# ardaduz/deep-video-mvs

Hardware: AMD Instinct MI355X
Metric: depth frames/sec/GPU @ 320x256x64 planes (fusionnet); rel-L1 vs ref (higher is better)
Workload: dtype f32

## Files before the change

### deep-video-mvs_amd/csrc/direct_conv.hip

```cpp
#include <stdlib.h>

#include "dvmvs_device.h"

namespace dvmvs {

typedef float float4v __attribute__((ext_vector_type(4)));

struct DirectConvArgs {
  const float* x;
  const float* packed;
  const float* bias;
  float* dst;
  float* dst_nhwc;
  long long x_batch_stride, dst_batch_stride;
  int B, C_in, C_out, H, W, OH, OW;
  int act;
  int n_groups;
  int packed_groups;
  int n_chunks;
  int tiles_x;
  int vec4;
};

#ifdef DVMVS_SWEEP_TRACE
constexpr int kDcTraceWords = 8, kDcTraceWaves = 16384;
// ... 308 lines not shown
  packed[i] = (kx < K && co < C_out && ci < C_in) ? w[((static_cast<size_t>(co) * C_in + ci) * K + ky) * K + kx] : 0.0f;
}

__device__ inline float head_activation(float v, int act, float p0, float p1) {
#pragma clang fp contract(off)
  if (act == 1) return fmaxf(v, 0.0f);
  if (act == 2 || act == 3) {
    const float s = 1.0f / (1.0f + expf(-v));
    return act == 2 ? s : 1.0f / (p0 * s + p1);
  }
  return v;
}

template <int PX>
__global__ __launch_bounds__(256) void conv_head_kernel(const float* __restrict__ x, const float* __restrict__ w, const float* __restrict__ bias,
                                                        float* __restrict__ dst, long long x_batch_stride, long long dst_batch_stride, int C, int H,
                                                        int W, int act, float p0, float p1) {
  constexpr int SL = 256 / PX;
  __shared__ float s_part[SL][PX];
  const int px = threadIdx.x % PX, slice = threadIdx.x / PX;
  const int HW = H * W;
  const int p = blockIdx.x * PX + px, b = blockIdx.y;
  const int y = p / W, xx = p - y * W;
  const int per = (C + SL - 1) / SL;
  const int c_lo = slice * per, c_hi = min(C, c_lo + per);
  float sum = 0.0f;
  if (p < HW) {
    int off[9];
    bool in[9];
#pragma unroll
    for (int t = 0; t < 9; ++t) {
      const int yy = y + t / 3 - 1, xs = xx + t % 3 - 1;
      in[t] = yy >= 0 && yy < H && xs >= 0 && xs < W;
      off[t] = in[t] ? yy * W + xs : 0;
    }
    const float* xb = x + static_cast<size_t>(b) * x_batch_stride;
#pragma unroll 2
    for (int c = c_lo; c < c_hi; ++c) {
      const float* plane = xb + static_cast<size_t>(c) * HW;
      float v[9];
#pragma unroll
      for (int t = 0; t < 9; ++t) v[t] = in[t] ? plane[off[t]] : 0.0f;
#pragma unroll
      for (int t = 0; t < 9; ++t) sum = fmaf(v[t], w[c * 9 + t], sum);
    }
  }
  s_part[slice][px] = sum;
  __syncthreads();
  if (slice == 0 && p < HW) {
    float total = s_part[0][px];
#pragma unroll
    for (int s = 1; s < SL; ++s) total += s_part[s][px];
    if (bias) total += bias[0];
    dst[static_cast<size_t>(b) * dst_batch_stride + p] = head_activation(total, act, p0, p1);
  }
}

struct DirectConvShape {
  int MW, MT, NT, PW, KS;
};
constexpr DirectConvShape kDcShapes[4] = {{16, 5, 2, 4, 2}, {8, 5, 2, 1, 8}, {16, 5, 1, 1, 8}, {8, 5, 1, 1, 8}};
constexpr int kDcCUs = 256;

inline int direct_conv_choose(int B, int C_in, int C_out, int H, int W, int K, int S) {
  if (B <= 0 || C_in <= 0 || C_out <= 0 || C_out % 16 != 0 || (K != 3 && K != 5) || (S != 1 && S != 2) || H <= 0 || W <= 0) return 0;
  if (S == 2 && (H % 2 != 0 || W % 2 != 0)) return 0;
  const int OH = H / S, OW = W / S;
#if defined(DVMVS_SWEEP_TUNING)
  const char* f = getenv("DVMVS_DC_SHAPE");
  const int forced = f ? atoi(f) : 0;
#else
  const int forced = 0;
#endif
  int best = 0;
  double best_fill = 0.0;
// ... 94 lines not shown
  a.dst_batch_stride = dst_batch_stride ? dst_batch_stride : static_cast<long long>(C_out) * a.OH * a.OW;
  if (a.x_batch_stride < static_cast<long long>(C_in) * H * W || a.dst_batch_stride < static_cast<long long>(C_out) * a.OH * a.OW) return DVMVS_EINVAL;
  if (W % 4 != 0 || a.x_batch_stride % 4 != 0 || (reinterpret_cast<uintptr_t>(x) & 15) != 0) return DVMVS_EUNSUPPORTED;
  if (static_cast<long long>(C_in + 64) * H * W * 4 >= (1LL << 31)) return DVMVS_EUNSUPPORTED;
  a.act = activation;
  a.n_groups = (C_in + 3) / 4;
  a.packed_groups = dc_packed_groups(C_in);
  a.vec4 = (a.OW % 4 == 0 && (a.OH * a.OW) % 4 == 0 && a.dst_batch_stride % 4 == 0 && (reinterpret_cast<uintptr_t>(dst) & 15) == 0) ? 1 : 0;
  a.n_chunks = 0; a.tiles_x = 0;
  hipStream_t s = static_cast<hipStream_t>(stream);
  if (kernel_size == 3) return stride == 1 ? launch_direct_conv_shape<3, 1>(id, a, s) : launch_direct_conv_shape<3, 2>(id, a, s);
  return stride == 1 ? launch_direct_conv_shape<5, 1>(id, a, s) : launch_direct_conv_shape<5, 2>(id, a, s);
}

extern "C" int dvmvs_conv_head_fwd(const float* x, long long x_batch_stride, const float* weight, const float* bias, float* dst,
                                   long long dst_batch_stride, int B, int C_in, int H, int W, int activation, float p0, float p1, dvmvs_stream_t stream) {
  using namespace dvmvs;
  if (!x || !weight || !dst || B <= 0 || C_in <= 0 || H <= 0 || W <= 0) return DVMVS_EINVAL;
  if (activation < 0 || activation > 3) return DVMVS_EINVAL;
  const long long HW = static_cast<long long>(H) * W;
  if (x_batch_stride == 0) x_batch_stride = HW * C_in;
  if (dst_batch_stride == 0) dst_batch_stride = HW;
  hipStream_t s = static_cast<hipStream_t>(stream);
  if (HW >= 16384) {
    hipLaunchKernelGGL((conv_head_kernel<64>), dim3(static_cast<unsigned int>((HW + 63) / 64), B), dim3(256), 0, s, x, weight, bias, dst, x_batch_stride,
                       dst_batch_stride, C_in, H, W, activation, p0, p1);
  } else {
    hipLaunchKernelGGL((conv_head_kernel<16>), dim3(static_cast<unsigned int>((HW + 15) / 16), B), dim3(256), 0, s, x, weight, bias, dst, x_batch_stride,
                       dst_batch_stride, C_in, H, W, activation, p0, p1);
  }
  return launch_status();
}

#ifdef DVMVS_SWEEP_TRACE
extern "C" int dvmvs_debug_direct_conv_trace(unsigned long long* host, int waves) {
  if (waves > dvmvs::kDcTraceWaves) waves = dvmvs::kDcTraceWaves;
  return static_cast<int>(hipMemcpyFromSymbol(host, HIP_SYMBOL(dvmvs::g_dc_trace), sizeof(unsigned long long) * dvmvs::kDcTraceWords * waves));
}
#endif
```

### deep-video-mvs_amd/csrc/frame_ops.hip

```cpp
#include "dvmvs_device.h"

namespace dvmvs {

template <int ACT>
__device__ inline float apply_act(float v, float p0 = 0.0f, float p1 = 0.0f) {
  if (ACT == 1) return fmaxf(v, 0.0f);
  if (ACT == 2) return 1.0f / (1.0f + expf(-v));
  if (ACT == 3) {
#pragma clang fp contract(off)
    const float s = 1.0f / (1.0f + expf(-v));
    return 1.0f / (p0 * s + p1);
  }
  return v;
}

template <int ACT, bool VEC4, int RES>
__global__ __launch_bounds__(256) void bias_act_kernel(const float* x, float* dst, long long dst_batch_stride, const float* __restrict__ bias,
                                                       const float* __restrict__ residual, int C, int HW, int W, float p0, float p1) {
  const int plane = blockIdx.y;
  const int b = plane / C, c = plane - b * C;
  const float bv = bias ? bias[c] : 0.0f;
  const float* p = x + static_cast<size_t>(plane) * HW;
  float* d = dst + static_cast<size_t>(b) * dst_batch_stride + static_cast<size_t>(c) * HW;
  if (VEC4 && RES != 2) {
// ... 86 lines not shown
      const float v00 = PRE ? apply_act<PRE>(r0[x0] + bv) : r0[x0], v01 = PRE ? apply_act<PRE>(r0[x1] + bv) : r0[x1];
      const float v10 = PRE ? apply_act<PRE>(r1[x0] + bv) : r1[x0], v11 = PRE ? apply_act<PRE>(r1[x1] + bv) : r1[x1];
      v[e] = h0 * (w0 * v00 + w1 * v01) + h1 * (w0 * v10 + w1 * v11);
    }
    *reinterpret_cast<float4v*>(dst + oy * OW + ox) = v;
  }
}

template <int PRE>
__global__ __launch_bounds__(256) void upsample2x_quads_kernel(const float* __restrict__ in, float* __restrict__ out, long long out_batch_stride,
                                                               const float* __restrict__ pre_bias, int C, int H, int W) {
  upsample2x_quads_plane<PRE>(in, out, out_batch_stride, pre_bias, blockIdx.y, C, H, W);
}

template <int PRE2>
__global__ __launch_bounds__(256) void upsample2x_pair_quads_kernel(const float* __restrict__ in1, float* __restrict__ out1, long long out1_batch_stride, int C1,
                                                                    const float* __restrict__ in2, float* __restrict__ out2, long long out2_batch_stride,
                                                                    const float* __restrict__ pre_bias2, int C2, int planes1, int H, int W) {
  const int pl = blockIdx.y;
  if (pl < planes1) upsample2x_quads_plane<0>(in1, out1, out1_batch_stride, nullptr, pl, C1, H, W);
  else upsample2x_quads_plane<PRE2>(in2, out2, out2_batch_stride, pre_bias2, pl - planes1, C2, H, W);
}

template <int K, int ACT, bool PRE>
__global__ __launch_bounds__(256) void depthwise_conv_kernel(const float* __restrict__ in, const float* __restrict__ weight,
                                                             const float* __restrict__ bias, const float* __restrict__ pre_bias,
                                                             float* __restrict__ out, int C, int H, int W, int OH, int OW, int stride) {
  const int c = blockIdx.y, b = blockIdx.z;
  const float* wk = weight + static_cast<size_t>(c) * K * K;
  const float* src = in + (static_cast<size_t>(b) * C + c) * H * W;
  float* dst = out + (static_cast<size_t>(b) * C + c) * OH * OW;
  const float bv = bias ? bias[c] : 0.0f;
  const float pv = (PRE && pre_bias) ? pre_bias[c] : 0.0f;
  for (int i = blockIdx.x * blockDim.x + threadIdx.x; i < OH * OW; i += gridDim.x * blockDim.x) {
    const int oy = i / OW, ox = i - oy * OW;
    const int y0 = oy * stride - K / 2, x0 = ox * stride - K / 2;
    float acc = 0.0f;
#pragma unroll
    for (int ky = 0; ky < K; ++ky) {
      const int y = y0 + ky;
      const bool yin = y >= 0 && y < H;
#pragma unroll
      for (int kx = 0; kx < K; ++kx) {
        const int x = x0 + kx;
        float v = 0.0f;
        if (yin && x >= 0 && x < W) v = PRE ? fmaxf(src[y * W + x] + pv, 0.0f) : src[y * W + x];
// ... 126 lines not shown
  using namespace dvmvs;
  if (!in1 || !out1 || !in2 || !out2 || B <= 0 || C1 <= 0 || C2 <= 0 || H <= 0 || W <= 0) return DVMVS_EINVAL;
  if (pre_activation2 < 0 || pre_activation2 > 2) return DVMVS_EINVAL;
  if (out1_batch_stride == 0) out1_batch_stride = static_cast<long long>(C1) * H * W * 4;
  if (out2_batch_stride == 0) out2_batch_stride = static_cast<long long>(C2) * H * W * 4;
  if (out1_batch_stride < static_cast<long long>(C1) * H * W * 4 || out2_batch_stride < static_cast<long long>(C2) * H * W * 4) return DVMVS_EINVAL;
  const long long planes = static_cast<long long>(B) * (C1 + C2);
  const bool quads = W % 2 == 0 && ((reinterpret_cast<uintptr_t>(out1) | reinterpret_cast<uintptr_t>(out2)) & 15) == 0 && ((out1_batch_stride | out2_batch_stride) & 3) == 0 &&
                     planes <= 65535 && static_cast<long long>(H) * W < (1LL << 27);
  if (!quads) {
    const int rc = dvmvs_upsample2x_fwd(in1, out1, out1_batch_stride, nullptr, 0, B, C1, H, W, stream);
    return rc != 0 ? rc : dvmvs_upsample2x_fwd(in2, out2, out2_batch_stride, pre_bias2, pre_activation2, B, C2, H, W, stream);
  }
  const int n_quads = 2 * H * (W / 2);
  const int per_plane = max(1, min((n_quads + 255) / 256, max(1, 4096 / static_cast<int>(planes))));
  const dim3 grid(static_cast<unsigned>(per_plane), static_cast<unsigned>(planes)), block(256);
  hipStream_t s = static_cast<hipStream_t>(stream);
#define DVMVS_UP2(P) hipLaunchKernelGGL(upsample2x_pair_quads_kernel<P>, grid, block, 0, s, in1, out1, out1_batch_stride, C1, in2, out2, out2_batch_stride, pre_bias2, C2, B * C1, H, W)
  if (pre_activation2 == 1) DVMVS_UP2(1); else if (pre_activation2 == 2) DVMVS_UP2(2); else DVMVS_UP2(0);
#undef DVMVS_UP2
  return launch_status();
}

extern "C" int dvmvs_depthwise_conv_fwd(const float* in, const float* weight, const float* bias, const float* pre_bias, int pre_relu,
                                        float* out, int B, int C, int H, int W, int kernel_size, int stride, int activation,
                                        dvmvs_stream_t stream) {
  using namespace dvmvs;
  if (!in || !weight || !out || B <= 0 || C <= 0 || H <= 0 || W <= 0) return DVMVS_EINVAL;
  if ((kernel_size != 3 && kernel_size != 5) || (stride != 1 && stride != 2) || activation < 0 || activation > 2) return DVMVS_EUNSUPPORTED;
  if (C > 65535 || B > 65535) return DVMVS_EUNSUPPORTED;
  const int pad = kernel_size / 2;
  const int OH = (H + 2 * pad - kernel_size) / stride + 1, OW = (W + 2 * pad - kernel_size) / stride + 1;
  hipStream_t s = static_cast<hipStream_t>(stream);
#define DVMVS_DW(K, A) return launch_depthwise<K, A>(in, weight, bias, pre_bias, pre_relu != 0, out, B, C, H, W, OH, OW, stride, s)
  if (kernel_size == 3) {
    if (activation == 0) DVMVS_DW(3, 0);
    if (activation == 1) DVMVS_DW(3, 1);
    DVMVS_DW(3, 2);
  }
  if (activation == 0) DVMVS_DW(5, 0);
  if (activation == 1) DVMVS_DW(5, 1);
  DVMVS_DW(5, 2);
#undef DVMVS_DW
}

extern "C" int dvmvs_nchw_to_nhwc(const float* src, float* dst, int B, int C, int H, int W, dvmvs_stream_t stream) {
// ... 27 lines not shown
```

### deep-video-mvs_amd/dvmvs/engine.py

```python
import contextlib
import copy
import time
import os
from collections import OrderedDict
from typing import NamedTuple

import torch
from torch import nn

from dvmvs.config import Config
from dvmvs.hip import ops as _ops
from dvmvs import pose_algebra as _pose_algebra
from dvmvs import utils as _utils

import dvmvs as _package
_DETERMINISTIC_MIOPEN = _package.DETERMINISTIC_MIOPEN
_MIOPEN_SWITCH_WAS_PRESET = _package.MIOPEN_SWITCH_WAS_PRESET or os.environ.get("DVMVS_KEEP_MIOPEN_ATOMIC_KERNELS", "0") == "1"

_MAX_MEAS = 8
_STAGING_SLOTS = int(os.environ.get("DVMVS_STAGING_SLOTS", "1"))
_GRAPH_QUEUE_FILLERS = int(os.environ.get("DVMVS_GRAPH_QUEUE_FILLERS", "1"))
def _fork_point(value):
    try:
        level = int(value)
# ... 575 lines not shown
        self.step_clock = None
        self._parity, self._prefetched = 0, None
        self._side_stream = torch.cuda.Stream(device=self.device)
        self._aux_stream = torch.cuda.Stream(device=self.device) if _AUX_STREAM != "0" else None
        self._planner, self._planned, self._param_host_ahead = None, None, None
        self.plan_frames_ahead = os.environ.get("DVMVS_PLAN_AHEAD", "1") != "0"
        self.planned_frames_used = 0
        self.ring_wait_seconds = 0.0
        self.lookahead_rejected = 0
        self._switch_interval_before = None
        self._filler_buffers, self._filler_graphs = None, []
        self._copies = CopyQueue()
        self._staging_seen = {}
        self.warm_captured_graphs = os.environ.get("DVMVS_WARM_GRAPHS", "1") != "0"
        self.warm_graph_launches = max(1, int(os.environ.get("DVMVS_WARM_GRAPH_LAUNCHES", "3")))
        if max_lookahead is None:
            max_lookahead = int(os.environ.get("DVMVS_LOOKAHEAD", "1"))
        self.max_lookahead = max(0, min(2, int(max_lookahead)))
        self.warmup_seconds = {"eager_first_frames": 0.0, "graph_capture": 0.0, "graph_first_launches": 0.0}
        self.warmup_graphs_launched = 0
        self.lstm_gates_on_partials = os.environ.get("DVMVS_LSTM_GATES_ON_PARTIALS", "1") != "0"
        self.sweep_variant_counts = {}
        self.sweep_work_list = bool(_utils.SWEEP_WORK_LIST and self.pose_algebra == "reference" and _utils.COST_VOLUME_VARIANT in (0, 2, 3, 4, 5))
        self.sweep_mfma = bool(self.direct and self.sweep_work_list and _utils.COST_VOLUME_VARIANT == 0 and os.environ.get("DVMVS_SWEEP_MFMA", "1") != "0"
                               and (self.height // 2) * (self.width // 2) >= 64 * 64)
        self._tiled_variants = (6,) if self.sweep_mfma else (2, 3, 4, 5)
        self._feature_cache = FeatureCache(self.cache_size, self.device, self.sweep_mfma)
        self.reset()

    def conv_plan_report(self):
        rows = []
        for m in (self.fe, self.fs, self.enc, self.lstm, self.dec):
            for sub in ([] if m is None else m.modules()):
                if isinstance(sub, FusedConv2d):
                    rows += [(shape, tuple(sub.weight.shape)) + tuple(plan) for shape, plan in sub.plans.items()]
        return rows

    @property
    def is_fusionnet(self):
        return self.lstm is not None

    def reset(self, sequence=None):
        if sequence is None or self.sequences == 1:
            self.has_previous = False
            self._no_previous[:] = True
            if self._static is not None:
# ... 256 lines not shown
        self._param_host.copy_(self._param_host_ahead)
        self.planned_frames_used += 1
        return result

    def _fpn_direct(self, taps, outs, half_nhwc=None):
        fpn = self.fs.fpn
        top = fpn.inner_blocks[-1](taps[-1])
        for level in range(len(taps) - 2, -1, -1):
            top = fpn.inner_blocks[level](taps[level], residual=top, residual_mode=2)
            if level == 0 and half_nhwc is not None and isinstance(fpn.layer_blocks[0], FusedConv2d):
                fpn.layer_blocks[0](top, out=outs[0], out_nhwc=half_nhwc)
                half_nhwc = None
            else:
                fpn.layer_blocks[level](top, out=outs[level])
        if half_nhwc is not None:
            _ops.nchw_to_nhwc_into(outs[0], half_nhwc)

    def _decoder_block_direct(self, block, x, cat, depth_head, depth_input):
        up_channels = block.up_convolution.conv[0].weight.shape[0]
        up_conv = block.up_convolution.conv[0]
        if depth_head is not None and _PAIRED_UPSAMPLING and self._aux_stream is None:
            B, C, H, W = x.shape
            up = torch.empty((B, C, 2 * H, 2 * W), device=x.device, dtype=torch.float32)
            _ops.upsample2x_pair_into(x, up, depth_head[0](depth_input, raw=True), cat[:, -1:], depth_head[0].bias, _ops.ACTIVATIONS["sigmoid"])
            up_conv(up, out=cat[:, :up_channels])
            return block.convolution2[0](block.convolution1[0](cat))
        if depth_head is not None:
            with self._beside("heads"):
                self._upsampled_depth_head(depth_head, depth_input, cat[:, -1:])
        if isinstance(up_conv, FusedConv2d):
            up_conv.forward_upsampled(x, out=cat[:, :up_channels])
        else:
            up_conv(_ops.upsample2x(x), out=cat[:, :up_channels])
        self._join_beside()
        return block.convolution2[0](block.convolution1[0](cat))

    @contextlib.contextmanager
    def _beside(self, use):
        aux = self._aux_stream if _AUX_STREAM in ("1", use) else None
        if aux is None:
            yield
            return
        aux.wait_stream(torch.cuda.current_stream(self.device))
        with torch.cuda.stream(aux):
            yield
        self._beside_open = True

    def _join_beside(self):
        if self._aux_stream is not None and getattr(self, "_beside_open", False):
            torch.cuda.current_stream(self.device).wait_stream(self._aux_stream)
            self._beside_open = False

    @staticmethod
    def _upsampled_depth_head(head, x, dst):
        _ops.upsample2x_into(head[0](x, raw=True), dst, head[0].bias, _ops.ACTIVATIONS["sigmoid"])

    def _lstm_bottleneck(self, x):
        if not self.bottleneck_convs:
# ... 121 lines not shown
            cell = self.lstm.lstm_cell
            if not state_warped:
                self._state_warp_direct(buffers, has_previous)
            self._join_beside()
            if self._lstm_bottleneck(lstm_cat):
                splits = _ops.bottleneck_conv_into(lstm_cat, self._lstm_packed, cell.conv.weight.shape[0], 1, self._lstm_partials)
                if self.lstm_gates_on_partials:
                    _ops.lstm_gates_partials_into(self._lstm_partials, splits, s["c"], s["h"])
                else:
                    _ops.partial_sums_bias_act_into(self._lstm_partials, splits, self._lstm_combined, None, _ops.ACTIVATIONS["none"],
                                                    tuple(self._lstm_combined.shape))
                    _ops.lstm_gates_into(self._lstm_combined, s["c"], s["h"])
            else:
                combined = cell.conv(lstm_cat)
                if not combined.is_contiguous():
                    combined = combined.contiguous()
                _ops.lstm_gates_into(combined, s["c"], s["h"])
            bottom = s["h"]
        d1 = self._decoder_block_direct(dec.decoder_block1, bottom, dec_cat[0], None, None)
        d2 = self._decoder_block_direct(dec.decoder_block2, d1, dec_cat[1], dec.depth_layer_one_sixteen, d1)
        d3 = self._decoder_block_direct(dec.decoder_block3, d2, dec_cat[2], dec.depth_layer_one_eight, d2)
        d4 = self._decoder_block_direct(dec.decoder_block4, d3, dec_cat[3], dec.depth_layer_quarter, d3)
        full_in = buffers["full_in"]
        if _PAIRED_UPSAMPLING and self._aux_stream is None:
            _ops.upsample2x_pair_into(d4, full_in[:, :32], dec.depth_layer_half[0](d4, raw=True), full_in[:, 32:33], dec.depth_layer_half[0].bias,
                                      _ops.ACTIVATIONS["sigmoid"])
        else:
            with self._beside("heads"):
                self._upsampled_depth_head(dec.depth_layer_half, d4, full_in[:, 32:33])
            _ops.upsample2x_into(d4, full_in[:, :32])
            self._join_beside()
        refined = dec.refine[1][0](dec.refine[0][0](full_in))
        dec.depth_layer_full[0](refined, out=s["prev_depth"], activation=_ops.ACTIVATION_SIGMOID_TO_DEPTH,
                                p0=dec.inverse_depth_multiplier, p1=dec.inverse_depth_base)

    def _frame_body(self, n_meas, has_previous, sweep_variant=0, parity=0, have=0, give=0, n_meas_next=0, next_variant=0):
        if self.direct:
            return self._frame_body_direct(n_meas, has_previous, sweep_variant, parity, have, give, n_meas_next, next_variant)
        s = self._static
        feats = self._features(s["image"])
        ref_half = feats[0].contiguous()
        s["ref_half"].copy_(ref_half)
        Hm, kt = self._sweep_views(n_meas)
        exact = self.pose_algebra == "exact"
        if exact:
            Hm, kt = _ops.sweep_matrices(s["pose"], s["meas_pose"][:n_meas], s["half_K"])
        cost_volume = _ops.cost_volume(ref_half, s["meas_feat"][:n_meas], Hm, kt, self.min_depth, self.max_depth, self.n_depth_levels,
# ... 269 lines not shown
```

### deep-video-mvs_amd/dvmvs/hip/_capi.py

```python
import ctypes
import os
import threading

import torch

_HERE = os.path.dirname(os.path.abspath(__file__))
LIB_PATH = os.environ.get("DVMVS_HIP_LIB", os.path.normpath(os.path.join(_HERE, "..", "..", "lib", "libdvmvs_hip.so")))

ABI_VERSION = 11
MAX_MEASUREMENTS = 8
MAX_DEPTH_LEVELS = 256
LAYOUT_NCHW, LAYOUT_NHWC = 0, 1

_c_fp = ctypes.c_void_p
_c_fpp = ctypes.POINTER(ctypes.c_void_p)
_c_int = ctypes.c_int
_c_dbl = ctypes.c_double
_c_stream = ctypes.c_void_p
_c_f3 = ctypes.POINTER(ctypes.c_float)

SIGNATURES = {
    "dvmvs_abi_version": (_c_int, []),
    "dvmvs_build_arch": (ctypes.c_char_p, []),
    "dvmvs_error_string": (ctypes.c_char_p, [_c_int]),
# ... 69 lines not shown
    "dvmvs_gp_filter_step": (_c_int, [_c_fp, _c_fp, _c_fp, _c_int, _c_dbl, _c_dbl, _c_dbl, _c_dbl, _c_dbl, _c_dbl, _c_int, _c_stream]),
    "dvmvs_dps_volume_fwd": (_c_int, [_c_fp, _c_fp, _c_fp, _c_fp, _c_fp, _c_fp, _c_int, _c_int, _c_int, _c_int, _c_int, _c_dbl, _c_stream]),
    "dvmvs_dps_regress_fwd": (_c_int, [_c_fp, _c_fp, _c_fp, _c_int, _c_int, _c_int, _c_int, _c_int, _c_int, _c_dbl, _c_stream]),
    "dvmvs_preprocess_rgb_fwd": (_c_int, [_c_fp, _c_fp, _c_int, _c_int, _c_int, ctypes.c_longlong, _c_int, _c_int, _c_int, _c_int,
                                          ctypes.c_longlong, _c_dbl, _c_f3, _c_f3, _c_int, _c_stream]),
    "dvmvs_preprocess_depth_fwd": (_c_int, [_c_fp, _c_fp, _c_int, _c_int, _c_int, _c_int, _c_int, _c_int, _c_int, _c_dbl, _c_stream]),
    "dvmvs_depth_errors_workspace_bytes": (ctypes.c_size_t, [_c_int, ctypes.c_longlong]),
    "dvmvs_depth_errors_fwd": (_c_int, [_c_fp, _c_fp, _c_int, ctypes.c_longlong, ctypes.c_float, _c_fp, _c_fp, _c_fp, _c_stream]),
    "dvmvs_tsdf_raycast_mask_bytes": (ctypes.c_size_t, [_c_int, _c_int, _c_int]),
    "dvmvs_tsdf_raycast_mask": (_c_int, [_c_fp, _c_fp, _c_int, _c_int, _c_int, _c_fp, _c_stream]),
    "dvmvs_tsdf_raycast_fwd": (_c_int, [_c_fp, _c_fp, _c_fp, _c_int, _c_int, _c_int, ctypes.c_float, ctypes.c_float, ctypes.c_float,
                                        ctypes.c_float, _c_fp, _c_fp, _c_fp, _c_int, _c_int, _c_int, ctypes.c_float, ctypes.c_float,
                                        ctypes.c_float, _c_fp, _c_fp, _c_fp, _c_stream]),
    "dvmvs_tsdf_integrate_frames_workspace_bytes": (ctypes.c_size_t, [_c_int]),
    "dvmvs_tsdf_integrate_frames": (_c_int, [_c_fp, _c_fp, _c_fp, _c_int, _c_int, _c_int, ctypes.c_float, ctypes.c_float, ctypes.c_float,
                                             ctypes.c_float, _c_fp, _c_fp, _c_fp, _c_fp, _c_fp, _c_int, _c_int, _c_int, ctypes.c_float,
                                             _c_f3, ctypes.c_float, _c_fp, _c_fp, _c_stream]),
    "dvmvs_nearest_workspace_bytes": (ctypes.c_size_t, [ctypes.c_longlong]),
    "dvmvs_nearest_query_workspace_bytes": (ctypes.c_size_t, [ctypes.c_longlong, ctypes.c_longlong]),
    "dvmvs_nearest_build": (_c_int, [_c_fp, ctypes.c_longlong, _c_fp, ctypes.c_size_t, _c_stream]),
    "dvmvs_nearest_distance_fwd": (_c_int, [_c_fp, ctypes.c_longlong, _c_fp, ctypes.c_longlong, _c_fp, _c_fp, ctypes.c_size_t, _c_fp, _c_fp,
                                            _c_stream]),
    "dvmvs_distance_metrics_fwd": (_c_int, [_c_fp, ctypes.c_longlong, _c_fp, ctypes.c_longlong, ctypes.c_float, _c_fp, _c_fp, _c_stream]),
}

ADDED_WITHIN_ABI = ("dvmvs_preprocess_rgb_fwd", "dvmvs_preprocess_depth_fwd")
ADDED_WITHIN_ABI_DEPTH_ERRORS = ("dvmvs_depth_errors_workspace_bytes", "dvmvs_depth_errors_fwd")
ADDED_WITHIN_ABI_TSDF_RAYCAST = ("dvmvs_tsdf_raycast_mask_bytes", "dvmvs_tsdf_raycast_mask", "dvmvs_tsdf_raycast_fwd")
ADDED_WITHIN_ABI_TSDF_FUSE = ("dvmvs_tsdf_integrate_frames_workspace_bytes", "dvmvs_tsdf_integrate_frames")
ADDED_WITHIN_ABI_NEAREST = ("dvmvs_nearest_workspace_bytes", "dvmvs_nearest_query_workspace_bytes", "dvmvs_nearest_build",
                            "dvmvs_nearest_distance_fwd", "dvmvs_distance_metrics_fwd")

_lib = None
_lock = threading.Lock()


def lib():
    global _lib
    if _lib is not None:
        return _lib
    with _lock:
        if _lib is not None:
            return _lib
        if not os.path.exists(LIB_PATH):
            raise RuntimeError(
                f"dvmvs HIP library not found at {LIB_PATH}. Build it with `make -C deep-video-mvs_amd/csrc` "
                f"(or __graft_entry__.build()). The plane-sweep ops have no CPU / eager fallback.")
        handle = ctypes.CDLL(LIB_PATH)
        added = (ADDED_WITHIN_ABI + ADDED_WITHIN_ABI_DEPTH_ERRORS + ADDED_WITHIN_ABI_TSDF_RAYCAST + ADDED_WITHIN_ABI_TSDF_FUSE
                 + ADDED_WITHIN_ABI_NEAREST)
        missing = [name for name in added if not hasattr(handle, name)]
        if missing:
            raise RuntimeError(f"{LIB_PATH} was built before {', '.join(missing)} joined ABI {ABI_VERSION} (the number did not change); "
                               f"rebuild it with `make -C deep-video-mvs_amd/csrc` (or __graft_entry__.build())")
        for name, (restype, argtypes) in SIGNATURES.items():
            fn = getattr(handle, name)
            fn.restype = restype
            fn.argtypes = argtypes
        got = handle.dvmvs_abi_version()
        if got != ABI_VERSION:
            raise RuntimeError(f"libdvmvs_hip.so ABI {got} does not match the Python binding ({ABI_VERSION}); rebuild")
        _lib = handle
    return _lib


def check(code, what):
    if code != 0:
        msg = lib().dvmvs_error_string(code).decode()
        raise RuntimeError(f"{what} failed with code {code}: {msg}")


def float_array(values):
    return (ctypes.c_float * len(values))(*[float(v) for v in values])
# ... 8 lines not shown
```

### deep-video-mvs_amd/dvmvs/hip/ops.py

```python
import ctypes
import os
from typing import Optional, Sequence, Tuple

import numpy as np
import torch
from torch import Tensor

from dvmvs.hip import _capi

__all__ = ["cost_volume", "sweep_matrices", "hidden_warp", "relative_pose", "lstm_gates", "depth_reproject", "depth_reproject_lowres",
           "bias_act_", "upsample2x", "depthwise_conv", "rgb_sweep", "gp_filter_step", "dps_volume", "dps_regress", "preprocess_rgb",
           "preprocess_depth", "depth_errors", "tsdf_raycast", "tsdf_raycast_mask", "tsdf_integrate_frames", "nearest_distance", "nearest_build",
           "nearest_query", "distance_metrics"]


COST_VOLUME_TWO_PASS = os.environ.get("DVMVS_COST_VOLUME_TWO_PASS", "1") == "1"


_workspaces = {}


def sweep_workspace(device, B, M, H, W, D):
    device = torch.device(device)
    index = device.index if device.index is not None else torch.cuda.current_device()
# ... 615 lines not shown
    with torch.cuda.device(x.device):
        rc = _capi.lib().dvmvs_upsample2x_fwd(_ptr(x), _ptr(dst), stride, _ptr(pre_bias) if pre_bias is not None and pre_bias.numel() else None,
                                              int(pre_activation), B, C, H, W, _stream(x))
    _capi.check(rc, "dvmvs_upsample2x_fwd")
    return dst


def upsample2x_pair_into(x1: Tensor, dst1: Tensor, x2: Tensor, dst2: Tensor, pre_bias2=None, pre_activation2: int = 0) -> None:
    _dev_f32("upsample2x_pair_into", x1, x2)
    x1, x2 = x1.contiguous(), x2.contiguous()
    B, C1, H, W = x1.shape
    C2 = x2.shape[1]
    if tuple(x2.shape) != (B, C2, H, W):
        raise ValueError(f"dvmvs::upsample2x_pair_into: the two maps must have the same batch and size, got {tuple(x1.shape)} and {tuple(x2.shape)}")
    stride1 = _slice_batch_stride("upsample2x_pair_into", dst1, B, C1, 2 * H, 2 * W)
    stride2 = _slice_batch_stride("upsample2x_pair_into", dst2, B, C2, 2 * H, 2 * W)
    if pre_bias2 is not None and pre_bias2.numel() not in (0, C2):
        raise ValueError(f"dvmvs::upsample2x_pair_into: pre_bias2 has {pre_bias2.numel()} entries for {C2} channels")
    with torch.cuda.device(x1.device):
        rc = _capi.lib().dvmvs_upsample2x_pair_fwd(_ptr(x1), _ptr(dst1), stride1, C1, _ptr(x2), _ptr(dst2), stride2,
                                                   _ptr(pre_bias2) if pre_bias2 is not None and pre_bias2.numel() else None, int(pre_activation2), C2, B, H, W,
                                                   _stream(x1))
    _capi.check(rc, "dvmvs_upsample2x_pair_fwd")


def lstm_gates_into(combined_conv: Tensor, c_state: Tensor, h_state: Tensor) -> None:
    _dev_f32("lstm_gates_into", combined_conv, c_state, h_state)
    B, hidden, H, W = c_state.shape
    if tuple(combined_conv.shape) != (B, 4 * hidden, H, W) or tuple(h_state.shape) != tuple(c_state.shape):
        raise ValueError("dvmvs::lstm_gates_into: shapes do not match")
    if not (combined_conv.is_contiguous() and c_state.is_contiguous() and h_state.is_contiguous()):
        raise ValueError("dvmvs::lstm_gates_into: expected contiguous tensors")
    with torch.cuda.device(c_state.device):
        rc = _capi.lib().dvmvs_lstm_gates_fwd(_ptr(combined_conv), _ptr(c_state), _ptr(h_state), _ptr(c_state), B, hidden, H, W, _stream(c_state))
    _capi.check(rc, "dvmvs_lstm_gates_fwd")


def bottleneck_conv_splits(B: int, C_out: int, C_in: int, H_in: int, W_in: int, stride: int) -> int:
    n = _capi.lib().dvmvs_bottleneck_conv_splits(int(B), int(C_out), int(C_in), int(H_in), int(W_in), int(stride))
    return n if n > 0 else 0


def bottleneck_conv_pack(weight: Tensor) -> Tensor:
    _dev_f32("bottleneck_conv_pack", weight)
    C_out, C_in, kh, kw = weight.shape
    nbytes = _capi.lib().dvmvs_bottleneck_conv_packed_bytes(C_out, C_in) if (kh, kw) == (3, 3) else 0
# ... 769 lines not shown
```

### include/dvmvs_hip.h

```cpp
#ifndef DVMVS_HIP_H
#define DVMVS_HIP_H

#include <stddef.h>
#include <stdint.h>

#ifdef __cplusplus
extern "C" {
#endif

#define DVMVS_ABI_VERSION 11
#define DVMVS_MAX_MEASUREMENTS 8
#define DVMVS_MAX_DEPTH_LEVELS 256

#define DVMVS_LAYOUT_NCHW 0
#define DVMVS_LAYOUT_NHWC 1

#define DVMVS_EINVAL (-1)
#define DVMVS_EUNSUPPORTED (-2)
#define DVMVS_ELIBRARY (-3)

typedef void* dvmvs_stream_t;

int dvmvs_abi_version(void);
const char* dvmvs_build_arch(void);
// ... 90 lines not shown
                             long long residual_batch_stride, int residual_mode, float* dst, long long dst_batch_stride, int B, int C_in,
                             int H, int W, int C_out, int activation, int splits, dvmvs_stream_t stream);

int dvmvs_depth_reproject_fwd(const float* transformation, const float* previous_depth, const float* full_K,
                              const float* half_K, float* out, float* out_lowres, int lowres_factor,
                              int B, int full_height, int full_width, dvmvs_stream_t stream);
int dvmvs_depth_reproject_lowres_fwd(const float* transformation, const float* previous_depth, const float* full_K,
                                     const float* half_K, float* zbuffer, float* out_lowres, int lowres_factor,
                                     int B, int full_height, int full_width, dvmvs_stream_t stream);

int dvmvs_depth_reproject_estimate_fwd(const float* transformation, const float* previous_depth, const float* full_K,
                                       const float* half_K, float* estimate, float* estimate_to_clear, int lowres_factor,
                                       int B, int full_height, int full_width, dvmvs_stream_t stream);

int dvmvs_bias_act_fwd(const float* x, float* dst, long long dst_batch_stride, const float* bias, const float* residual,
                       int residual_mode, int B, int C, int H, int W, int activation, float p0, float p1, dvmvs_stream_t stream);
int dvmvs_bias_act_inplace(float* x, const float* bias, const float* residual, int residual_mode, int B, int C, int H, int W,
                           int activation, dvmvs_stream_t stream);
int dvmvs_upsample2x_fwd(const float* in, float* out, long long out_batch_stride, const float* pre_bias, int pre_activation,
                         int B, int C, int H, int W, dvmvs_stream_t stream);
int dvmvs_upsample2x_pair_fwd(const float* in1, float* out1, long long out1_batch_stride, int C1, const float* in2, float* out2,
                              long long out2_batch_stride, const float* pre_bias2, int pre_activation2, int C2, int B, int H, int W,
                              dvmvs_stream_t stream);
int dvmvs_conv_bias_act_fwd(const float* x, const float* weight, const float* bias, float* out, long long out_batch_stride,
                            int B, int Cin, int H, int W, int Cout, int K, int stride, int padding, int activation, dvmvs_stream_t stream);
int dvmvs_depthwise_conv_fwd(const float* in, const float* weight, const float* bias, const float* pre_bias, int pre_relu, float* out,
                             int B, int C, int H, int W, int kernel_size, int stride, int activation, dvmvs_stream_t stream);

int dvmvs_tsdf_integrate(float* tsdf_vol, float* weight_vol, float* color_vol, int dim_x, int dim_y, int dim_z,
                         float origin_x, float origin_y, float origin_z, float voxel_size, const float* cam_intr,
                         const float* cam_pose, const float* color_im, const float* depth_im, int im_h, int im_w,
                         float trunc_margin, float obs_weight, dvmvs_stream_t stream);

size_t dvmvs_marching_cubes_workspace_bytes(int X, int Y, int Z);
int dvmvs_marching_cubes_count(const float* vol, int X, int Y, int Z, float level, void* workspace, size_t workspace_bytes,
                               long long* counts_dev, dvmvs_stream_t stream);
int dvmvs_marching_cubes_emit(const float* vol, const float* color_vol, int X, int Y, int Z, float level, float ox, float oy, float oz,
                              float voxel_size, void* workspace, float* verts, float* normals, unsigned char* colors, int* faces,
                              long long V, long long F, dvmvs_stream_t stream);

int dvmvs_rgb_sweep_fwd(const float* image1, const float* const* image2s, const float* Hm, const float* kt, float* out,
                        int B, int M, int C, int H, int W, int D, double min_depth, double max_depth, int Cout,
                        int channel_offset, int copy_image, dvmvs_stream_t stream);
int dvmvs_gp_filter_step(double* state, const float* y, float* z, int N, double a00, double a01, double a10, double a11,
                         double k0, double k1, int reset, dvmvs_stream_t stream);

// ... 43 lines not shown
```

Before: 1411.

## Fuse decoder depth head conv, sigmoid and bilinear upsample into one tail kernel

Adds a decoder_tail kernel that computes the 1-channel 3x3 depth head conv on a low-res tile staged through shared memory, applies sigmoid, and bilinearly upsamples to full resolution. The same grid also carries the feature-map 2x upsample planes. This replaces the separate conv_head launch plus paired upsample and drops the intermediate low-res head buffer round trip. The cost is extra halo recomputation per tile and a more complex tiling plan, with the old path kept as a fallback.

```diff
diff --git a/deep-video-mvs_amd/csrc/conv_head.h b/deep-video-mvs_amd/csrc/conv_head.h
--- /dev/null
+++ b/deep-video-mvs_amd/csrc/conv_head.h
@@ -0,0 +1,55 @@
+#pragma once
+
+#include "dvmvs_device.h"
+
+namespace dvmvs {
+
+template <int SL>
+__device__ inline void head_slice_range(int slice, int C, int& c_lo, int& c_hi) {
+  const int per = (C + SL - 1) / SL;
+  c_lo = slice * per;
+  c_hi = min(C, c_lo + per);
+}
+
+__device__ inline float head_channel_fma(float sum, const float (&v)[9], const float* __restrict__ w9) {
+#pragma unroll
+  for (int t = 0; t < 9; ++t) sum = fmaf(v[t], w9[t], sum);
+  return sum;
+}
+
+template <int SL>
+__device__ inline float head_slice_sum(const float* __restrict__ xb, const float* __restrict__ w, int slice, int y, int xx, int C, int H, int W) {
+  const int HW = H * W;
+  int c_lo, c_hi;
+  head_slice_range<SL>(slice, C, c_lo, c_hi);
+  int off[9];
+  bool in[9];
+#pragma unroll
+  for (int t = 0; t < 9; ++t) {
+    const int yy = y + t / 3 - 1, xs = xx + t % 3 - 1;
+    in[t] = yy >= 0 && yy < H && xs >= 0 && xs < W;
+    off[t] = in[t] ? yy * W + xs : 0;
+  }
+  float sum = 0.0f;
+#pragma unroll 2
+  for (int c = c_lo; c < c_hi; ++c) {
+    const float* plane = xb + static_cast<size_t>(c) * HW;
+    float v[9];
+#pragma unroll
+    for (int t = 0; t < 9; ++t) v[t] = in[t] ? plane[off[t]] : 0.0f;
+    sum = head_channel_fma(sum, v, w + c * 9);
+  }
+  return sum;
+}
+
+template <int SL>
+__device__ inline float head_add_slices(const float* column, int stride) {
+  float total = column[0];
+#pragma unroll
+  for (int s = 1; s < SL; ++s) total += column[s * stride];
+  return total;
+}
+
+inline bool head_four_slices(long long HW) { return HW >= 16384; }
+
+}
diff --git a/deep-video-mvs_amd/csrc/direct_conv.hip b/deep-video-mvs_amd/csrc/direct_conv.hip
--- a/deep-video-mvs_amd/csrc/direct_conv.hip
+++ b/deep-video-mvs_amd/csrc/direct_conv.hip
@@ -1,6 +1,7 @@
 #include <stdlib.h>
 
 #include "dvmvs_device.h"
+#include "conv_head.h"
 
 namespace dvmvs {
 
@@ -355,35 +356,10 @@
   const int HW = H * W;
   const int p = blockIdx.x * PX + px, b = blockIdx.y;
   const int y = p / W, xx = p - y * W;
-  const int per = (C + SL - 1) / SL;
-  const int c_lo = slice * per, c_hi = min(C, c_lo + per);
-  float sum = 0.0f;
-  if (p < HW) {
-    int off[9];
-    bool in[9];
-#pragma unroll
-    for (int t = 0; t < 9; ++t) {
-      const int yy = y + t / 3 - 1, xs = xx + t % 3 - 1;
-      in[t] = yy >= 0 && yy < H && xs >= 0 && xs < W;
-      off[t] = in[t] ? yy * W + xs : 0;
-    }
-    const float* xb = x + static_cast<size_t>(b) * x_batch_stride;
-#pragma unroll 2
-    for (int c = c_lo; c < c_hi; ++c) {
-      const float* plane = xb + static_cast<size_t>(c) * HW;
-      float v[9];
-#pragma unroll
-      for (int t = 0; t < 9; ++t) v[t] = in[t] ? plane[off[t]] : 0.0f;
-#pragma unroll
-      for (int t = 0; t < 9; ++t) sum = fmaf(v[t], w[c * 9 + t], sum);
-    }
-  }
-  s_part[slice][px] = sum;
+  s_part[slice][px] = p < HW ? head_slice_sum<SL>(x + static_cast<size_t>(b) * x_batch_stride, w, slice, y, xx, C, H, W) : 0.0f;
   __syncthreads();
   if (slice == 0 && p < HW) {
-    float total = s_part[0][px];
-#pragma unroll
-    for (int s = 1; s < SL; ++s) total += s_part[s][px];
+    float total = head_add_slices<SL>(&s_part[0][px], PX);
     if (bias) total += bias[0];
     dst[static_cast<size_t>(b) * dst_batch_stride + p] = head_activation(total, act, p0, p1);
   }
@@ -524,7 +500,7 @@
   if (x_batch_stride == 0) x_batch_stride = HW * C_in;
   if (dst_batch_stride == 0) dst_batch_stride = HW;
   hipStream_t s = static_cast<hipStream_t>(stream);
-  if (HW >= 16384) {
+  if (head_four_slices(HW)) {
     hipLaunchKernelGGL((conv_head_kernel<64>), dim3(static_cast<unsigned int>((HW + 63) / 64), B), dim3(256), 0, s, x, weight, bias, dst, x_batch_stride,
                        dst_batch_stride, C_in, H, W, activation, p0, p1);
   } else {
diff --git a/deep-video-mvs_amd/csrc/frame_ops.hip b/deep-video-mvs_amd/csrc/frame_ops.hip
--- a/deep-video-mvs_amd/csrc/frame_ops.hip
+++ b/deep-video-mvs_amd/csrc/frame_ops.hip
@@ -1,4 +1,8 @@
+#include <stdio.h>
+#include <stdlib.h>
+
 #include "dvmvs_device.h"
+#include "conv_head.h"
 
 namespace dvmvs {
 
@@ -132,6 +136,154 @@
   else upsample2x_quads_plane<PRE2>(in2, out2, out2_batch_stride, pre_bias2, pl - planes1, C2, H, W);
 }
 
+template <int SL_, int KC_, int PP_, int NPASS_>
+struct TailConfig {
+  static constexpr int SL = SL_, KC = KC_, PP = PP_, NPASS = NPASS_;
+  static constexpr int PX = 256 / SL, NCH = SL * KC, STRIDE = PP + 4;
+  static constexpr int NLOAD = NCH * PP / 256, NW = (NCH * 9 + 255) / 256;
+  static_assert(256 % PP == 0 && NCH % (256 / PP) == 0, "a thread stages one window position of every (256 / PP)-th channel");
+  static constexpr bool takes(int toh, int tow) {
+    return toh > 0 && tow > 0 && tow % 4 == 0 && ((toh - 1) / 2 + 3) * ((tow - 1) / 2 + 3) <= PX * NPASS && ((toh - 1) / 2 + 5) * ((tow - 1) / 2 + 5) <= PP;
+  }
+};
+typedef TailConfig<16, 8, 64, 1> TailTinyMaps;
+typedef TailConfig<16, 4, 64, 3> TailSmallMaps;
+typedef TailConfig<4, 8, 128, 1> TailLargeMaps;
+static_assert(TailTinyMaps::takes(4, 4) && TailSmallMaps::takes(8, 8) && TailLargeMaps::takes(8, 16), "the launcher's tiles");
+
+template <class Cfg>
+__device__ inline void decoder_tail_depth_tile(const float* __restrict__ x, const float* __restrict__ w, const float* __restrict__ bias, float* __restrict__ depth,
+                                               long long depth_batch_stride, int tile, int C, int H, int W, int toh, int tow) {
+#pragma clang fp contract(off)
+  typedef float float4v __attribute__((ext_vector_type(4)));
+  constexpr int SL = Cfg::SL, KC = Cfg::KC, PP = Cfg::PP, PX = Cfg::PX, NPASS = Cfg::NPASS, STRIDE = Cfg::STRIDE;
+  __shared__ float s_x[Cfg::NCH * STRIDE];
+  __shared__ float s_w[Cfg::NCH * 9];
+  __shared__ float s_part[SL][PX];
+  __shared__ float s_act[PX * NPASS];
+  const int OH = 2 * H, OW = 2 * W, HW = H * W;
+  const float sh = OH > 1 ? static_cast<float>(H - 1) / static_cast<float>(OH - 1) : 0.0f;
+  const float sw = OW > 1 ? static_cast<float>(W - 1) / static_cast<float>(OW - 1) : 0.0f;
+  const int tiles_x = (OW + tow - 1) / tow, tiles_y = (OH + toh - 1) / toh;
+  const int b = tile / (tiles_x * tiles_y), t = tile - b * (tiles_x * tiles_y);
+  const int ty = t / tiles_x, tx = t - ty * tiles_x;
+  const int oy_lo = ty * toh, oy_hi = min(OH, oy_lo + toh), ox_lo = tx * tow, ox_hi = min(OW, ox_lo + tow);
+  const int sy_lo = static_cast<int>(sh * static_cast<float>(oy_lo)), sx_lo = static_cast<int>(sw * static_cast<float>(ox_lo));
+  const int ly0 = static_cast<int>(sh * static_cast<float>(oy_hi - 1)), lx0 = static_cast<int>(sw * static_cast<float>(ox_hi - 1));
+  const int sy_hi = ly0 + (ly0 < H - 1 ? 1 : 0), sx_hi = lx0 + (lx0 < W - 1 ? 1 : 0);
+  const int src_w = sx_hi - sx_lo + 1, n_src = src_w * (sy_hi - sy_lo + 1);
+  const int pw = src_w + 2, n_patch = pw * (sy_hi - sy_lo + 3);
+  if (n_src > PX * NPASS || n_patch > PP) return;
+  const float* xb = x + static_cast<size_t>(b) * C * HW;
+  const int per = (C + SL - 1) / SL;
+
+  const int pos = threadIdx.x % PP, chl0 = threadIdx.x / PP;
+  const int wy = sy_lo - 1 + pos / pw, wx = sx_lo - 1 + pos % pw;
+  const bool pos_in = pos < n_patch && wy >= 0 && wy < H && wx >= 0 && wx < W;
+  const int pos_off = pos_in ? wy * W + wx : 0;
+  float rx[Cfg::NLOAD], rw[Cfg::NW];
+  auto fetch = [&](int j0) {
+#pragma unroll
+    for (int k = 0; k < Cfg::NLOAD; ++k) {
+      const int chl = chl0 + k * (256 / PP);
+      const int j = j0 + chl / SL, c = (chl % SL) * per + j;
+      rx[k] = (pos_in && j < per && c < C) ? xb[static_cast<size_t>(c) * HW + pos_off] : 0.0f;
+    }
+#pragma unroll
+    for (int k = 0; k < Cfg::NW; ++k) {
+      const int idx = threadIdx.x + k * 256;
+      const int chl = idx / 9;
+      const int j = j0 + chl / SL, c = (chl % SL) * per + j;
+      rw[k] = (chl < Cfg::NCH && j < per && c < C) ? w[c * 9 + idx % 9] : 0.0f;
+    }
+  };
+
+  const int px = threadIdx.x % PX, slice = threadIdx.x / PX;
+  int c_lo, c_hi;
+  head_slice_range<SL>(slice, C, c_lo, c_hi);
+  int tap0[NPASS];
+  float sum[NPASS];
+#pragma unroll
+  for (int p = 0; p < NPASS; ++p) {
+    const int i = min(p * PX + px, n_src - 1);
+    const int ry = i / src_w;
+    tap0[p] = ry * pw + (i - ry * src_w);
+    sum[p] = 0.0f;
+  }
+  fetch(0);
+  for (int j0 = 0; j0 < per; j0 += KC) {
+    __syncthreads();
+#pragma unroll
+    for (int k = 0; k < Cfg::NLOAD; ++k) s_x[(chl0 + k * (256 / PP)) * STRIDE + pos] = rx[k];
+#pragma unroll
+    for (int k = 0; k < Cfg::NW; ++k)
+      if (threadIdx.x + k * 256 < Cfg::NCH * 9) s_w[threadIdx.x + k * 256] = rw[k];
+    __syncthreads();
+    if (j0 + KC < per) fetch(j0 + KC);
+#pragma unroll
+    for (int p = 0; p < NPASS; ++p) {
+      if (p * PX < n_src) {
+#pragma unroll
+        for (int j = 0; j < KC; ++j) {
+          const float* plane = s_x + (j * SL + slice) * STRIDE + tap0[p];
+          float v[9];
+#pragma unroll
+          for (int tp = 0; tp < 9; ++tp) v[tp] = plane[(tp / 3) * pw + tp % 3];
+          const float next = head_channel_fma(sum[p], v, s_w + (j * SL + slice) * 9);
+          sum[p] = c_lo + j0 + j < c_hi ? next : sum[p];
+        }
+      }
+    }
+  }
+  const float bv = bias ? bias[0] : 0.0f;
+#pragma unroll
+  for (int p = 0; p < NPASS; ++p) {
+    if (p * PX < n_src) {
+      const int i = p * PX + px;
+      __syncthreads();
+      s_part[slice][px] = sum[p];
+      __syncthreads();
+      if (slice == 0 && i < n_src) s_act[i] = apply_act<2>(head_add_slices<SL>(&s_part[0][px], PX) + bv);
+    }
+  }
+  __syncthreads();
+  float* dst = depth + static_cast<size_t>(b) * depth_batch_stride;
+  const int qw = (ox_hi - ox_lo) >> 2;
+  for (int q = threadIdx.x; q < (oy_hi - oy_lo) * qw; q += 256) {
+    const int qy = q / qw;
+    const int oy = oy_lo + qy, ox = ox_lo + 4 * (q - qy * qw);
+    const float fy = sh * static_cast<float>(oy);
+    const int y0 = static_cast<int>(fy);
+    const int y1 = y0 + (y0 < H - 1 ? 1 : 0);
+    const float h1 = fy - static_cast<float>(y0), h0 = 1.0f - h1;
+    const int r0 = (y0 - sy_lo) * src_w - sx_lo, r1 = (y1 - sy_lo) * src_w - sx_lo;
+    float4v v;
+#pragma unroll
+    for (int e = 0; e < 4; ++e) {
+      const float fx = sw * static_cast<float>(ox + e);
+      const int x0 = static_cast<int>(fx);
+      const int x1 = x0 + (x0 < W - 1 ? 1 : 0);
+      const float w1 = fx - static_cast<float>(x0), w0 = 1.0f - w1;
+      const float v00 = s_act[r0 + x0], v01 = s_act[r0 + x1], v10 = s_act[r1 + x0], v11 = s_act[r1 + x1];
+      v[e] = h0 * (w0 * v00 + w1 * v01) + h1 * (w0 * v10 + w1 * v11);
+    }
+    *reinterpret_cast<float4v*>(dst + oy * OW + ox) = v;
+  }
+}
+
+template <class Cfg>
+__global__ __launch_bounds__(256) void decoder_tail_kernel(const float* __restrict__ x, float* __restrict__ up, long long up_batch_stride, const float* __restrict__ w,
+                                                           const float* __restrict__ bias, float* __restrict__ depth, long long depth_batch_stride,
+                                                           int depth_rows, int depth_tiles, int C, int H, int W, int toh, int tow) {
+  const int row = blockIdx.y;
+  if (row >= depth_rows) {
+    upsample2x_quads_plane<0>(x, up, up_batch_stride, nullptr, row - depth_rows, C, H, W);
+    return;
+  }
+  const int tile = row * gridDim.x + blockIdx.x;
+  if (tile < depth_tiles) decoder_tail_depth_tile<Cfg>(x, w, bias, depth, depth_batch_stride, tile, C, H, W, toh, tow);
+}
+
 template <int K, int ACT, bool PRE>
 __global__ __launch_bounds__(256) void depthwise_conv_kernel(const float* __restrict__ in, const float* __restrict__ weight,
                                                              const float* __restrict__ bias, const float* __restrict__ pre_bias,
@@ -304,6 +456,82 @@
   return launch_status();
 }
 
+namespace dvmvs {
+
+constexpr int kDecoderTailCUs = 256;
+
+struct DecoderTailPlan {
+  bool fused, four_slices;
+  int config;
+  int toh, tow, per_plane, depth_rows, depth_tiles;
+};
+
+inline DecoderTailPlan decoder_tail_plan(const float* up, long long up_batch_stride, const float* depth, long long depth_batch_stride, int B, int C, int H, int W) {
+  DecoderTailPlan p = {};
+  const long long planes = static_cast<long long>(B) * (C + 1);
+  if (W % 2 != 0 || ((reinterpret_cast<uintptr_t>(up) | reinterpret_cast<uintptr_t>(depth)) & 15) != 0 || ((up_batch_stride | depth_batch_stride) & 3) != 0 ||
+      planes > 65535 || static_cast<long long>(H) * W >= (1LL << 27))
+    return p;
+  p.four_slices = head_four_slices(static_cast<long long>(H) * W);
+  if (p.four_slices) {
+    p.toh = 8;
+    p.tow = 16;
+  } else {
+    const bool small = static_cast<long long>(B) * ((2 * H + 3) / 4) * ((2 * W + 3) / 4) <= 2 * kDecoderTailCUs;
+    p.toh = p.tow = small ? 4 : 8;
+  }
+#if defined(DVMVS_SWEEP_TUNING)
+  const char* f = getenv("DVMVS_TAIL_TILE");
+  int r = 0, c = 0;
+  if (f && sscanf(f, "%dx%d", &r, &c) == 2 && (p.four_slices ? TailLargeMaps::takes(r, c) : TailSmallMaps::takes(r, c))) {
+    p.toh = r;
+    p.tow = c;
+  }
+#endif
+  p.config = p.four_slices ? 2 : (TailTinyMaps::takes(p.toh, p.tow) ? 0 : 1);
+  const int n_quads = 2 * H * (W / 2);
+  p.per_plane = max(1, min((n_quads + 255) / 256, max(1, 4096 / static_cast<int>(planes))));
+  const long long tiles = static_cast<long long>(B) * ((2 * H + p.toh - 1) / p.toh) * ((2 * W + p.tow - 1) / p.tow);
+  const long long rows = (tiles + p.per_plane - 1) / p.per_plane;
+  if (rows + static_cast<long long>(B) * C > 65535) return p;
+  p.depth_tiles = static_cast<int>(tiles);
+  p.depth_rows = static_cast<int>(rows);
+  p.fused = true;
+  return p;
+}
+
+}
+
+extern "C" size_t dvmvs_decoder_tail_workspace_bytes(const float* up, long long up_batch_stride, const float* depth, long long depth_batch_stride, int B,
+                                                     int C, int H, int W) {
+  if (B <= 0 || C <= 0 || H <= 0 || W <= 0) return 0;
+  if (up_batch_stride == 0) up_batch_stride = static_cast<long long>(C) * H * W * 4;
+  if (depth_batch_stride == 0) depth_batch_stride = static_cast<long long>(H) * W * 4;
+  return dvmvs::decoder_tail_plan(up, up_batch_stride, depth, depth_batch_stride, B, C, H, W).fused ? 0 : sizeof(float) * B * H * W;
+}
+
+extern "C" int dvmvs_decoder_tail_fwd(const float* x, const float* head_weight, const float* head_bias, float* up, long long up_batch_stride, float* depth,
+                                      long long depth_batch_stride, float* workspace, int B, int C, int H, int W, dvmvs_stream_t stream) {
+  using namespace dvmvs;
+  if (!x || !head_weight || !up || !depth || B <= 0 || C <= 0 || H <= 0 || W <= 0) return DVMVS_EINVAL;
+  if (up_batch_stride == 0) up_batch_stride = static_cast<long long>(C) * H * W * 4;
+  if (depth_batch_stride == 0) depth_batch_stride = static_cast<long long>(H) * W * 4;
+  if (up_batch_stride < static_cast<long long>(C) * H * W * 4 || depth_batch_stride < static_cast<long long>(H) * W * 4) return DVMVS_EINVAL;
+  const DecoderTailPlan p = decoder_tail_plan(up, up_batch_stride, depth, depth_batch_stride, B, C, H, W);
+  if (!p.fused) {
+    if (!workspace) return DVMVS_EINVAL;
+    const int rc = dvmvs_conv_head_fwd(x, 0, head_weight, nullptr, workspace, 0, B, C, H, W, 0, 0.0f, 0.0f, stream);
+    return rc != 0 ? rc : dvmvs_upsample2x_pair_fwd(x, up, up_batch_stride, C, workspace, depth, depth_batch_stride, head_bias, 2, 1, B, H, W, stream);
+  }
+  const dim3 grid(static_cast<unsigned>(p.per_plane), static_cast<unsigned>(p.depth_rows + B * C)), block(256);
+  hipStream_t s = static_cast<hipStream_t>(stream);
+#define DVMVS_TAIL(CFG) hipLaunchKernelGGL(decoder_tail_kernel<CFG>, grid, block, 0, s, x, up, up_batch_stride, head_weight, head_bias, depth, depth_batch_stride, \
+                                          p.depth_rows, p.depth_tiles, C, H, W, p.toh, p.tow)
+  if (p.config == 2) DVMVS_TAIL(TailLargeMaps); else if (p.config == 1) DVMVS_TAIL(TailSmallMaps); else DVMVS_TAIL(TailTinyMaps);
+#undef DVMVS_TAIL
+  return launch_status();
+}
+
 extern "C" int dvmvs_depthwise_conv_fwd(const float* in, const float* weight, const float* bias, const float* pre_bias, int pre_relu,
                                         float* out, int B, int C, int H, int W, int kernel_size, int stride, int activation,
                                         dvmvs_stream_t stream) {
diff --git a/deep-video-mvs_amd/dvmvs/engine.py b/deep-video-mvs_amd/dvmvs/engine.py
--- a/deep-video-mvs_amd/dvmvs/engine.py
+++ b/deep-video-mvs_amd/dvmvs/engine.py
@@ -621,6 +621,7 @@
         self.lstm_gates_on_partials = os.environ.get("DVMVS_LSTM_GATES_ON_PARTIALS", "1") != "0"
         self.sweep_variant_counts = {}
         self.sweep_work_list = bool(_utils.SWEEP_WORK_LIST and self.pose_algebra == "reference" and _utils.COST_VOLUME_VARIANT in (0, 2, 3, 4, 5))
+        self.decoder_tail = os.environ.get("DVMVS_DECODER_TAIL", "1") != "0"
         self.sweep_mfma = bool(self.direct and self.sweep_work_list and _utils.COST_VOLUME_VARIANT == 0 and os.environ.get("DVMVS_SWEEP_MFMA", "1") != "0"
                                and (self.height // 2) * (self.width // 2) >= 64 * 64)
         self._tiled_variants = (6,) if self.sweep_mfma else (2, 3, 4, 5)
@@ -923,7 +924,10 @@
         if depth_head is not None and _PAIRED_UPSAMPLING and self._aux_stream is None:
             B, C, H, W = x.shape
             up = torch.empty((B, C, 2 * H, 2 * W), device=x.device, dtype=torch.float32)
-            _ops.upsample2x_pair_into(x, up, depth_head[0](depth_input, raw=True), cat[:, -1:], depth_head[0].bias, _ops.ACTIVATIONS["sigmoid"])
+            if depth_input is x and self._decoder_tail_takes(depth_head[0], x):
+                _ops.decoder_tail_into(x, up, depth_head[0].weight, depth_head[0].bias, cat[:, -1:])
+            else:
+                _ops.upsample2x_pair_into(x, up, depth_head[0](depth_input, raw=True), cat[:, -1:], depth_head[0].bias, _ops.ACTIVATIONS["sigmoid"])
             up_conv(up, out=cat[:, :up_channels])
             return block.convolution2[0](block.convolution1[0](cat))
         if depth_head is not None:
@@ -935,6 +939,11 @@
             up_conv(_ops.upsample2x(x), out=cat[:, :up_channels])
         self._join_beside()
         return block.convolution2[0](block.convolution1[0](cat))
+
+    def _decoder_tail_takes(self, head, x):
+        return (self.decoder_tail and isinstance(head, FusedConv2d) and head.direct_conv and not head.depthwise and head.groups == 1
+                and tuple(head.weight.shape) == (1, x.shape[1], 3, 3) and tuple(head.stride) == (1, 1) and tuple(head.padding) == (1, 1)
+                and tuple(head.dilation) == (1, 1) and x.is_contiguous() and x.data_ptr() % 16 == 0)
 
     @contextlib.contextmanager
     def _beside(self, use):
@@ -1102,7 +1111,9 @@
         d3 = self._decoder_block_direct(dec.decoder_block3, d2, dec_cat[2], dec.depth_layer_one_eight, d2)
         d4 = self._decoder_block_direct(dec.decoder_block4, d3, dec_cat[3], dec.depth_layer_quarter, d3)
         full_in = buffers["full_in"]
-        if _PAIRED_UPSAMPLING and self._aux_stream is None:
+        if _PAIRED_UPSAMPLING and self._aux_stream is None and self._decoder_tail_takes(dec.depth_layer_half[0], d4):
+            _ops.decoder_tail_into(d4, full_in[:, :32], dec.depth_layer_half[0].weight, dec.depth_layer_half[0].bias, full_in[:, 32:33])
+        elif _PAIRED_UPSAMPLING and self._aux_stream is None:
             _ops.upsample2x_pair_into(d4, full_in[:, :32], dec.depth_layer_half[0](d4, raw=True), full_in[:, 32:33], dec.depth_layer_half[0].bias,
                                       _ops.ACTIVATIONS["sigmoid"])
         else:
diff --git a/deep-video-mvs_amd/dvmvs/hip/_capi.py b/deep-video-mvs_amd/dvmvs/hip/_capi.py
--- a/deep-video-mvs_amd/dvmvs/hip/_capi.py
+++ b/deep-video-mvs_amd/dvmvs/hip/_capi.py
@@ -115,6 +115,8 @@
     "dvmvs_nearest_distance_fwd": (_c_int, [_c_fp, ctypes.c_longlong, _c_fp, ctypes.c_longlong, _c_fp, _c_fp, ctypes.c_size_t, _c_fp, _c_fp,
                                             _c_stream]),
     "dvmvs_distance_metrics_fwd": (_c_int, [_c_fp, ctypes.c_longlong, _c_fp, ctypes.c_longlong, ctypes.c_float, _c_fp, _c_fp, _c_stream]),
+    "dvmvs_decoder_tail_workspace_bytes": (ctypes.c_size_t, [_c_fp, ctypes.c_longlong, _c_fp, ctypes.c_longlong] + [_c_int] * 4),
+    "dvmvs_decoder_tail_fwd": (_c_int, [_c_fp, _c_fp, _c_fp, _c_fp, ctypes.c_longlong, _c_fp, ctypes.c_longlong, _c_fp] + [_c_int] * 4 + [_c_stream]),
 }
 
 ADDED_WITHIN_ABI = ("dvmvs_preprocess_rgb_fwd", "dvmvs_preprocess_depth_fwd")
@@ -123,6 +125,7 @@
 ADDED_WITHIN_ABI_TSDF_FUSE = ("dvmvs_tsdf_integrate_frames_workspace_bytes", "dvmvs_tsdf_integrate_frames")
 ADDED_WITHIN_ABI_NEAREST = ("dvmvs_nearest_workspace_bytes", "dvmvs_nearest_query_workspace_bytes", "dvmvs_nearest_build",
                             "dvmvs_nearest_distance_fwd", "dvmvs_distance_metrics_fwd")
+ADDED_WITHIN_ABI_DECODER_TAIL = ("dvmvs_decoder_tail_workspace_bytes", "dvmvs_decoder_tail_fwd")
 
 _lib = None
 _lock = threading.Lock()
@@ -141,7 +144,7 @@
                 f"(or __graft_entry__.build()). The plane-sweep ops have no CPU / eager fallback.")
         handle = ctypes.CDLL(LIB_PATH)
         added = (ADDED_WITHIN_ABI + ADDED_WITHIN_ABI_DEPTH_ERRORS + ADDED_WITHIN_ABI_TSDF_RAYCAST + ADDED_WITHIN_ABI_TSDF_FUSE
-                 + ADDED_WITHIN_ABI_NEAREST)
+                 + ADDED_WITHIN_ABI_NEAREST + ADDED_WITHIN_ABI_DECODER_TAIL)
         missing = [name for name in added if not hasattr(handle, name)]
         if missing:
             raise RuntimeError(f"{LIB_PATH} was built before {', '.join(missing)} joined ABI {ABI_VERSION} (the number did not change); "
diff --git a/deep-video-mvs_amd/dvmvs/hip/ops.py b/deep-video-mvs_amd/dvmvs/hip/ops.py
--- a/deep-video-mvs_amd/dvmvs/hip/ops.py
+++ b/deep-video-mvs_amd/dvmvs/hip/ops.py
@@ -661,6 +661,30 @@
                                                    _ptr(pre_bias2) if pre_bias2 is not None and pre_bias2.numel() else None, int(pre_activation2), C2, B, H, W,
                                                    _stream(x1))
     _capi.check(rc, "dvmvs_upsample2x_pair_fwd")
+
+
+def decoder_tail_into(x: Tensor, up: Tensor, head_weight: Tensor, head_bias, depth_dst: Tensor) -> None:
+    _dev_f32("decoder_tail_into", x, up, head_weight, depth_dst)
+    if x.dim() != 4 or not x.is_contiguous() or tuple(head_weight.shape) != (1, x.shape[1], 3, 3) or not head_weight.is_contiguous():
+        raise ValueError(f"dvmvs::decoder_tail_into: expected a contiguous NCHW input and a [1,{x.shape[1] if x.dim() == 4 else '?'},3,3] weight, "
+                         f"got {tuple(x.shape)}, {tuple(head_weight.shape)}")
+    B, C, H, W = x.shape
+    up_stride = _slice_batch_stride("decoder_tail_into", up, B, C, 2 * H, 2 * W)
+    depth_stride = _slice_batch_stride("decoder_tail_into", depth_dst, B, 1, 2 * H, 2 * W)
+    if head_bias is not None and head_bias.numel() not in (0, 1):
+        raise ValueError(f"dvmvs::decoder_tail_into: head_bias has {head_bias.numel()} entries for one channel")
+    if head_bias is not None and head_bias.numel():
+        _dev_f32("decoder_tail_into", head_bias)
+    if len({t.device for t in (x, up, head_weight, depth_dst)}) != 1:
+        raise ValueError("dvmvs::decoder_tail_into: the tensors are on different devices")
+    with torch.cuda.device(x.device):
+        library = _capi.lib()
+        nbytes = library.dvmvs_decoder_tail_workspace_bytes(_ptr(up), up_stride, _ptr(depth_dst), depth_stride, B, C, H, W)
+        workspace = torch.empty(nbytes // 4, device=x.device, dtype=torch.float32) if nbytes else None
+        rc = library.dvmvs_decoder_tail_fwd(_ptr(x), _ptr(head_weight), _ptr(head_bias) if head_bias is not None and head_bias.numel() else None, _ptr(up),
+                                            up_stride, _ptr(depth_dst), depth_stride, _ptr(workspace) if workspace is not None else None, B, C, H, W,
+                                            _stream(x))
+    _capi.check(rc, "dvmvs_decoder_tail_fwd")
 
 
 def lstm_gates_into(combined_conv: Tensor, c_state: Tensor, h_state: Tensor) -> None:
diff --git a/include/dvmvs_hip.h b/include/dvmvs_hip.h
--- a/include/dvmvs_hip.h
+++ b/include/dvmvs_hip.h
@@ -136,6 +136,10 @@
 int dvmvs_upsample2x_pair_fwd(const float* in1, float* out1, long long out1_batch_stride, int C1, const float* in2, float* out2,
                               long long out2_batch_stride, const float* pre_bias2, int pre_activation2, int C2, int B, int H, int W,
                               dvmvs_stream_t stream);
+size_t dvmvs_decoder_tail_workspace_bytes(const float* up, long long up_batch_stride, const float* depth, long long depth_batch_stride, int B,
+                                          int C, int H, int W);
+int dvmvs_decoder_tail_fwd(const float* x, const float* head_weight, const float* head_bias, float* up, long long up_batch_stride, float* depth,
+                           long long depth_batch_stride, float* workspace, int B, int C, int H, int W, dvmvs_stream_t stream);
 int dvmvs_conv_bias_act_fwd(const float* x, const float* weight, const float* bias, float* out, long long out_batch_stride,
                             int B, int Cin, int H, int W, int Cout, int K, int stride, int padding, int activation, dvmvs_stream_t stream);
 int dvmvs_depthwise_conv_fwd(const float* in, const float* weight, const float* bias, const float* pre_bias, int pre_relu, float* out,
```

After: 1376. 0.976x the previous value.
